# mmurooka/SMPLpp

Hardware: AMD Instinct MI355X
Metric: SMPL FK evals/s + IK iters/s, batch 1024 frames, 1/2/4/8 MI355X (higher is better)
Workload: dtype f32 (exact operands: every fp32 value as three bf16 pieces = fp32's 24 bits on the bf16 matrix pipe, fp32 accumulate; fp32 VALU skinning)

## Files before the change

smplpp_amd/csrc/skin_h.hip:

```cpp
#include "common.h"
#include "slot_pipe.h"

namespace smplpp_hip
{
typedef float f32x16 __attribute__((ext_vector_type(16)));
typedef float v3f __attribute__((ext_vector_type(3), aligned(4)));
typedef float v4f __attribute__((ext_vector_type(4)));
typedef unsigned v3u __attribute__((ext_vector_type(3)));
typedef _Float16 f16x8 __attribute__((ext_vector_type(8)));

constexpr int H_R = 7;
constexpr int H_LDS_RING = HB_G_BYTES;
constexpr int H_LDS_TR = H_LDS_RING + H_R * HB_IMG;
constexpr int H_LDS_TOTAL = H_LDS_TR + 64 * 16;

constexpr int wrap15(int u)
{
  return u < 0 ? u + HB_SLOTS : u;
}
constexpr int h_tail_slot(int k)
{
  return k <= 4 ? k : (k == 5 ? 4 : (k <= 10 ? k - 1 : (k == 11 ? 9 : k - 2)));
}
constexpr int h_tail_m(int k)
{
  return (k == 5 || k == 11) ? 8 : 5;
}
constexpr int h_tail_rows_in(int u)
{
  int c = 0;
  for(int k = 0; k < 16; k++) c += h_tail_slot(k) == u;
  return c;
}
constexpr int h_after_dma(int u, bool ht, bool rest)
{
  return u < 14 ? (ht ? h_tail_rows_in(u) : (u < 9 ? 2 : 0)) : ((u == 14 && rest) ? 16 : 0);
}
constexpr int h_slot_ops(int u, bool ht, bool rest)
{
  return 3 + h_after_dma(u, ht, rest);
}
constexpr int h_barrier_vmcnt(int s, bool ht, bool rest)
{
  if(!ht && s == 13) return 12;
  int c = s - 6 < 0 ? ((wrap15(s - 6) == 14 && rest && ht) ? 16 : 0) : h_after_dma(s - 6, ht, rest);
  for(int u = s - 5; u < s; u++) c += u < 0 ? 3 + ((wrap15(u) == 14 && rest && ht) ? 16 : 0) : h_slot_ops(u, ht, rest);
  return c < 63 ? c : 63;
}
static_assert(h_tail_rows_in(4) == 2 && h_tail_rows_in(9) == 2 && h_tail_rows_in(13) == 1 && h_tail_rows_in(14) == 0, "tail placement");
static_assert(h_barrier_vmcnt(0, false, true) == 15 && h_barrier_vmcnt(1, false, false) == 12 + 5 && h_barrier_vmcnt(0, true, true) == 31 &&
                  h_barrier_vmcnt(1, true, false) == 5 * 3 + 1 && h_barrier_vmcnt(8, true, false) == 15 + 7 && h_barrier_vmcnt(14, false, false) == 2 + 15,
              "window bookkeeping");

#ifndef SKINH_STORE_AUX
#define SKINH_STORE_AUX 0
#endif
#ifndef SKINH_DMA_IMM
#define SKINH_DMA_IMM 1
#endif
#ifndef SKINH_ABL
#define SKINH_ABL 0
#endif
#if SKINH_ABL & (256 | 512)
__device__ unsigned long long g_hslot_times[8 * 256];
__device__ unsigned long long g_hwg_times[256 * 4];
#endif

template<bool WANT_REST>
__global__ __launch_bounds__(256, 1) void skin_kernel_h(const uint8_t * __restrict__ A2h, const uint8_t * __restrict__ B2h,
                                                        const uint8_t * __restrict__ G2h, const float * __restrict__ theta,
                                                        float * __restrict__ verts, float * __restrict__ rest, int64_t n,
                                                        int64_t V, int nvg, int nft, float cAB)
{
  extern __shared__ __attribute__((aligned(16))) unsigned char lds[];
  typedef __attribute__((address_space(3))) void * lds_ptr_t;
  const int tid = threadIdx.x, lane = tid & 63, half = lane >> 5, l31 = lane & 31;
  const int wave = __builtin_amdgcn_readfirstlane(tid >> 6), wf = wave & 1, wv = wave >> 1;
  const int nbx = (int)(gridDim.x >> 3), xcd = (int)(blockIdx.x & 7), jb = (int)(blockIdx.x >> 3);
  const int vg0 = (xcd * nvg) >> 3, vg1 = ((xcd + 1) * nvg) >> 3, nvx = vg1 - vg0;
  const int cnt = nvx * nft;
  const int i0 = (int)(((unsigned)jb * (unsigned)cnt) / (unsigned)nbx), i1 = (int)(((unsigned)(jb + 1) * (unsigned)cnt) / (unsigned)nbx);
  if(i0 >= i1) return;

#if SKINH_ABL & 512
  const unsigned long long t_start = __builtin_amdgcn_s_memtime(), r_start = __builtin_amdgcn_s_memrealtime();
#endif
  const int frameB = (int)(V * 12);
  const __amdgpu_buffer_rsrc_t rsB =
      __builtin_amdgcn_make_buffer_rsrc(const_cast<uint8_t *>(B2h), 0, (int)(nvg * HB_SLOTS * HB_IMG), 0x00020000);
  const __amdgpu_buffer_rsrc_t rsG =
      __builtin_amdgcn_make_buffer_rsrc(const_cast<uint8_t *>(G2h), 0, (int)(nft * HB_G_BYTES), 0x00020000);
  const __amdgpu_buffer_rsrc_t rsV = __builtin_amdgcn_make_buffer_rsrc(verts, 0, (int)(verts ? n * V * 12 : 0), 0x00020000);
  const __amdgpu_buffer_rsrc_t rsR = __builtin_amdgcn_make_buffer_rsrc(rest, 0, (int)(rest ? n * V * 12 : 0), 0x00020000);
  const int voffDma = wave * 3072 + lane * 16;

  const unsigned char * imgV[H_R];
  int imgS[H_R];
#pragma unroll
  for(int k = 0; k < H_R; k++)
  {
    imgS[k] = H_LDS_RING + k * HB_IMG;
    imgV[k] = lds + imgS[k] + wv * 6144 + lane * 16;
  }
  const unsigned char * const gLane0 = lds + wf * (12 * 3072) + lane * 16;
  const unsigned char * const gLane1 = lds + wf * (12 * 3072) + 2048 + l31 * 16;
  const unsigned char * const trLane = lds + H_LDS_TR + (wf * 32 + 4 * half) * 16;

#if SKINH_ABL & (256 | 512)
  int dbg_item = 0;
#endif
  f32x16 acc[3], macc[3];
  float tt[3][16];
  v4f areg[HB_KS][2];
  v4f bfr[2][3][2];
  v4f gfr[2][4];
  v4f wfr[4];
  v4f trb[2];
  const f32x16 zero16 = {0.f, 0.f, 0.f, 0.f, 0.f, 0.f, 0.f, 0.f, 0.f, 0.f, 0.f, 0.f, 0.f, 0.f, 0.f, 0.f};

  struct Item
  {
    int voff;
    int sb;
    float cw;
  } cur = {0x7fffff00, 0, 0.f}, prev = {0x7fffff00, 0, 0.f};

  auto mfma = [](const v4f & a, const v4f & b, const f32x16 & c) {
    return __builtin_amdgcn_mfma_f32_32x32x16_f16(__builtin_bit_cast(f16x8, a), __builtin_bit_cast(f16x8, b), c, 0, 0, 0);
  };
  auto dma = [&](auto itag, int vgBase, int slot, int dst) {
    constexpr int I = decltype(itag)::value;
    if constexpr(SKINH_ABL & 2) return;
#if SKINH_DMA_IMM
    __builtin_amdgcn_raw_ptr_buffer_load_lds(rsB, (lds_ptr_t)(lds + dst + wave * 3072), 16, voffDma, vgBase + slot * HB_IMG, I * 1024, 0);
#else
    __builtin_amdgcn_raw_ptr_buffer_load_lds(rsB, (lds_ptr_t)(lds + dst + wave * 3072 + I * 1024), 16, voffDma,
                                             vgBase + slot * HB_IMG + I * 1024, 0, 0);
#endif
  };

  v3f ovh;
  auto tail_prep = [&](auto rtag) {
    constexpr int R = decltype(rtag)::value;
    const v4f tr = trb[R & 1];
    if constexpr(R + 1 < 16) trb[(R + 1) & 1] = *reinterpret_cast<const v4f *>(trLane + ((((R + 1) & 3) + 8 * ((R + 1) >> 2)) * 16));
    const float u = __builtin_fmaf(tt[2][R], cAB, macc[2][R]);
    ovh = v3f{__builtin_fmaf(tt[0][R], prev.cw, tr.x), __builtin_fmaf(tt[1][R], prev.cw, tr.y), __builtin_fmaf(u, prev.cw, tr.z)};
  };
  auto tail_store = [&](auto rtag) {
    constexpr int R = decltype(rtag)::value;
    constexpr int ROWC = (R & 3) + 8 * (R >> 2);
    if constexpr(SKINH_ABL & 32)
    {
      const float o0 = ovh.x, o1 = ovh.y, o2 = ovh.z;
      asm volatile("" ::"v"(o0), "v"(o1), "v"(o2));
    }
    else
      __builtin_amdgcn_raw_buffer_store_b96(__builtin_bit_cast(v3u, ovh), rsV, prev.voff, prev.sb + ROWC * frameB, SKINH_STORE_AUX);
    asm volatile("s_nop 1");
  };
  auto tail_row = [&](auto rtag) {
    tail_prep(rtag);
    tail_store(rtag);
  };
  auto standalone_tail = [&]() {
    static_for<16>([&](auto rr) {
      tail_row(rr);
      SCHED_BARRIER();
    });
  };

  auto load_frame_tile = [&](int ft, auto first_tag) {
    constexpr bool FIRST = decltype(first_tag)::value;
    full_barrier();
#if SKINH_ABL & 512
    if(FIRST && blockIdx.x == 8 && tid == 0) g_hslot_times[70] = __builtin_amdgcn_s_memtime();
#endif
    float tval = 0.0f;
    if(tid < 192)
    {
      const int64_t f = (int64_t)ft * 64 + tid / 3;
      if(f < n) tval = theta[f * ((NJ + 1) * 3) + tid % 3];
    }
    const int vgF = vg0 + i0 % nvx;
    if constexpr(FIRST)
    {
      dma(std::integral_constant<int, 0>{}, vgF * (HB_SLOTS * HB_IMG), 0, imgS[0]);
      dma(std::integral_constant<int, 1>{}, vgF * (HB_SLOTS * HB_IMG), 0, imgS[0]);
      dma(std::integral_constant<int, 2>{}, vgF * (HB_SLOTS * HB_IMG), 0, imgS[0]);
    }
    const uint8_t * ap = A2h + ((int64_t)ft * HB_KS * 2 + wf) * 2048 + lane * 16;
#pragma unroll
    for(int ks = 0; ks < HB_KS; ks++)
#pragma unroll
      for(int p = 0; p < 2; p++) areg[ks][p] = *reinterpret_cast<const v4f *>(ap + ks * HB_A_BYTES + p * 1024);
    if constexpr(FIRST)
      static_for<H_R - 1>([&](auto dd) {
        constexpr int D = decltype(dd)::value + 1;
        dma(std::integral_constant<int, 0>{}, vgF * (HB_SLOTS * HB_IMG), D, imgS[D]);
        dma(std::integral_constant<int, 1>{}, vgF * (HB_SLOTS * HB_IMG), D, imgS[D]);
        dma(std::integral_constant<int, 2>{}, vgF * (HB_SLOTS * HB_IMG), D, imgS[D]);
      });
    if constexpr(FIRST)
    {
      waitcnt_barrier<28 + 18, 0, !(SKINH_ABL & 1)>();
#pragma unroll
      for(int q = 0; q < 6; q++) bfr[0][q / 2][q % 2] = *reinterpret_cast<const v4f *>(imgV[0] + q * 1024);
    }
    if(tid < 192) *reinterpret_cast<float *>(lds + H_LDS_TR + (tid / 3) * 16 + (tid % 3) * 4) = tval;
#if SKINH_ABL & 512
    if(FIRST && blockIdx.x == 8 && tid == 0) g_hslot_times[72] = __builtin_amdgcn_s_memtime();
#endif
  };

  auto do_item = [&](int ft_in, int vg_in, int vgn_in, auto ht_tag) {
    constexpr bool HT = decltype(ht_tag)::value;
    const int ft = __builtin_amdgcn_readfirstlane(ft_in), vg = __builtin_amdgcn_readfirstlane(vg_in), vgn = __builtin_amdgcn_readfirstlane(vgn_in);
    const int Bcur = vg * (HB_SLOTS * HB_IMG), Bnext = vgn * (HB_SLOTS * HB_IMG);
    cur.sb = __builtin_amdgcn_readfirstlane((ft * 64 + wf * 32) * frameB);
    int gcls = 3;

#if SKINH_ABL & 512
    if(blockIdx.x == 8 && tid == 0 && dbg_item < 8)
    {
      g_hslot_times[dbg_item * 8 + 0] = __builtin_amdgcn_s_memtime();
      g_hslot_times[dbg_item * 8 + 1] = __builtin_amdgcn_s_memrealtime();
    }
#endif
    static_for<HB_KS>([&](auto ss) {
      constexpr int S = decltype(ss)::value;
      static_for<9>([&](auto mm) {
        constexpr int M = decltype(mm)::value, X = M / 3, Q = M % 3;
        const v4f & a = areg[S][Q == 2 ? 1 : 0];
        const v4f & b = bfr[S & 1][X][Q == 1 ? 1 : 0];
#if SKINH_ABL & 256
        if(blockIdx.x == 0 && tid == 0 && dbg_item < 8) g_hslot_times[dbg_item * 256 + S * 9 + M] = __builtin_readcyclecounter();
#endif
#if SKINH_ABL & 512
        if(M == 0 && S < 8 && blockIdx.x == 8 && tid == 0 && dbg_item == 0) g_hslot_times[80 + S] = __builtin_amdgcn_s_memtime();
#endif
        if constexpr(SKINH_ABL & 4)
        {
          if constexpr(S == 0 && Q == 0) acc[X] = zero16;
          asm volatile("" ::"v"(a), "v"(b));
        }
        else if constexpr(S == 0 && Q == 0)
          acc[X] = mfma(a, b, zero16);
        else
          acc[X] = mfma(a, b, acc[X]);
        SCHED_BARRIER();
        if constexpr(M == 1) waitcnt_barrier<h_barrier_vmcnt(S, HT, WANT_REST), 0, !(SKINH_ABL & 1)>();
        if constexpr(M >= 2 && M <= 4)
          dma(std::integral_constant<int, M - 2>{}, S + 7 < HB_SLOTS ? Bcur : Bnext, S + 7 < HB_SLOTS ? S + 7 : S + 7 - HB_SLOTS,
              imgS[S % H_R]);
        if constexpr(!HT && S < 9 && (M == 5 || M == 6))
        {
          constexpr int PC = (2 * S + (M - 5)) * 4;
          __builtin_amdgcn_raw_ptr_buffer_load_lds(rsG, (lds_ptr_t)(lds + (PC + wave) * 1024), 16, lane * 16,
                                                   ft * HB_G_BYTES + (PC + wave) * 1024, 0, 0);
        }
        if constexpr(HT && (M == 5 || M == 7))
          static_for<16>([&](auto kk) {
            constexpr int K = decltype(kk)::value;
            if constexpr(h_tail_slot(K) == S && h_tail_m(K) == (M == 5 ? 5 : 8)) tail_prep(kk);
          });
        if constexpr(HT && (M == 6 || M == 8))
          static_for<16>([&](auto kk) {
            constexpr int K = decltype(kk)::value;
            if constexpr(h_tail_slot(K) == S && h_tail_m(K) == (M == 6 ? 5 : 8)) tail_store(kk);
          });
        if constexpr(S < HB_KS - 1 && M >= 2 && M <= 4 && !(SKINH_ABL & 16))
        {
          bfr[(S + 1) & 1][M - 2][0] = *reinterpret_cast<const v4f *>(imgV[(S + 1) % H_R] + (2 * (M - 2)) * 1024);
          bfr[(S + 1) & 1][M - 2][1] = *reinterpret_cast<const v4f *>(imgV[(S + 1) % H_R] + (2 * (M - 2) + 1) * 1024);
        }
        if constexpr(S == HB_KS - 1)
        {
          const unsigned char * wimg = imgV[HB_KS % H_R] - wv * 4096;
          if constexpr(M >= 2 && M <= 5) wfr[M - 2] = *reinterpret_cast<const v4f *>(wimg + ((M - 2) / 2) * 4096 + ((M - 2) % 2) * 1024);
          if constexpr(M == 6)
          {
            cur.cw = *reinterpret_cast<const float *>(lds + imgS[HB_KS % H_R] + HB_CW_OFF + (wv * 32 + l31) * 4);
            const int pv = *reinterpret_cast<const int *>(lds + imgS[HB_KS % H_R] + HB_PERM_OFF + (wv * 32 + l31) * 4);
            cur.voff = pv >= 0 ? pv * 12 + (4 * half) * frameB : 0x7fffff00;
            gcls = __builtin_amdgcn_readfirstlane(*reinterpret_cast<const int *>(lds + imgS[HB_KS % H_R] + HB_FLAGS_OFF));
          }
          if constexpr(M == 7)
          {
            gfr[0][0] = *reinterpret_cast<const v4f *>(gLane0);
            gfr[0][1] = *reinterpret_cast<const v4f *>(gLane0 + 1024);
          }
          if constexpr(M == 8)
          {
            gfr[0][2] = *reinterpret_cast<const v4f *>(gLane1);
            gfr[0][3] = *reinterpret_cast<const v4f *>(gLane1 + 512);
          }
        }
        SCHED_BARRIER();
      });
    });

#if SKINH_ABL & 512
    if(blockIdx.x == 8 && tid == 0 && dbg_item < 8)
    {
      g_hslot_times[dbg_item * 8 + 2] = __builtin_amdgcn_s_memtime();
      g_hslot_times[dbg_item * 8 + 3] = __builtin_amdgcn_s_memrealtime();
    }
#endif
    auto skin_phase = [&](auto ctag) {
    constexpr int CLS = decltype(ctag)::value;
    constexpr bool K0 = (CLS & 1) != 0, K1 = (CLS & 2) != 0;
    static_for<12>([&](auto ee) {
      constexpr int E = decltype(ee)::value, MPE = E & 1, ME = E % 3;
      static_for<5>([&](auto bb) {
        constexpr int B = decltype(bb)::value;
        constexpr bool LIVE = (B == 0 || B == 1 || B == 3) ? K0 : K1;
        constexpr int FIRST = K0 ? 0 : 2;
        constexpr int GI = B < 2 ? 0 : (B == 2 ? 2 : (B == 3 ? 1 : 3));
        constexpr int WI = B == 0 ? 0 : (B == 1 ? 1 : (B == 2 ? 3 : (B == 3 ? 0 : 2)));
#if SKINH_ABL & 256
        if(blockIdx.x == 0 && tid == 0 && dbg_item < 8) g_hslot_times[dbg_item * 256 + 126 + E * 5 + B] = __builtin_readcyclecounter();
#endif
        if constexpr(SKINH_ABL & 8)
        {
          if constexpr(B == 0) macc[ME] = zero16;
        }
        else if constexpr(!LIVE)
          ;
        else if constexpr(B == FIRST)
          macc[ME] = mfma(gfr[MPE][GI], wfr[WI], zero16);
        else
          macc[ME] = mfma(gfr[MPE][GI], wfr[WI], macc[ME]);
        SCHED_BARRIER();
        if constexpr(E == 0 && B == 0) waitcnt_barrier<h_barrier_vmcnt(HB_KS, HT, WANT_REST), 0, !(SKINH_ABL & 1)>();
        if constexpr(E == 0 && B >= 1 && B <= 3) dma(std::integral_constant<int, B - 1>{}, Bnext, HB_KS + 7 - HB_SLOTS, imgS[HB_KS % H_R]);
        if constexpr(E == 1)
        {
          bfr[0][B / 2][B % 2] = *reinterpret_cast<const v4f *>(imgV[(HB_KS + 1) % H_R] + B * 1024);
          if constexpr(B == 4) bfr[0][2][1] = *reinterpret_cast<const v4f *>(imgV[(HB_KS + 1) % H_R] + 5 * 1024);
        }
        if constexpr(E < 11 && B <= 3 && !(SKINH_ABL & (8 | 16)))
        {
          constexpr int I = B == 0 ? 0 : (B == 1 ? 2 : (B == 2 ? 1 : 3));
          if constexpr(I < 2 ? K0 : K1)
            gfr[MPE ^ 1][I] = *reinterpret_cast<const v4f *>((I < 2 ? gLane0 + I * 1024 : gLane1 + (I - 2) * 512) + (E + 1) * 3072);
        }
        if constexpr(E == 11 && B == 4)
          trb[0] = *reinterpret_cast<const v4f *>(trLane);
        auto blend_rows = [&](auto ftag, auto r0tag, auto r1tag) {
          constexpr int F = decltype(ftag)::value, XF = F / 4, CF = F % 4, MF = F % 3, R0 = decltype(r0tag)::value, R1 = decltype(r1tag)::value;
#pragma unroll
          for(int r = R0; r < R1; r++)
          {
            if constexpr(CF == 0) tt[XF][r] = macc[MF][r] * acc[0][r];
            if constexpr(CF == 1) tt[XF][r] = __builtin_fmaf(macc[MF][r], acc[1][r], tt[XF][r]);
            if constexpr(CF == 2) tt[XF][r] = __builtin_fmaf(macc[MF][r], acc[2][r], tt[XF][r]);
            if constexpr(CF == 3) tt[XF][r] = __builtin_fmaf(tt[XF][r], cAB, macc[MF][r]);
          }
        };
        if constexpr(!(SKINH_ABL & 8))
        {
          if constexpr(E >= 1 && B >= 1)
            blend_rows(std::integral_constant<int, E - 1>{}, std::integral_constant<int, 3 * (B - 1)>{}, std::integral_constant<int, 3 * B>{});
          if constexpr(E >= 2 && B == 0)
            blend_rows(std::integral_constant<int, E - 2>{}, std::integral_constant<int, 12>{}, std::integral_constant<int, 16>{});
          if constexpr(E == 11 && B == 4)
            blend_rows(std::integral_constant<int, 10>{}, std::integral_constant<int, 12>{}, std::integral_constant<int, 16>{});
        }
        if constexpr(WANT_REST && E >= 2 && E <= 9 && B < 2)
        {
          constexpr int R = 2 * (E - 2) + B, ROWC = (R & 3) + 8 * (R >> 2);
          v3f ov = {acc[0][R] * cAB, acc[1][R] * cAB, acc[2][R] * cAB};
          __builtin_amdgcn_raw_buffer_store_b96(__builtin_bit_cast(v3u, ov), rsR, cur.voff, cur.sb + ROWC * frameB, SKINH_STORE_AUX);
          asm volatile("s_nop 1");
        }
        SCHED_BARRIER();
      });
    });
    };
    if(gcls == 1)
      skin_phase(std::integral_constant<int, 1>{});
    else if(gcls == 2)
      skin_phase(std::integral_constant<int, 2>{});
    else
      skin_phase(std::integral_constant<int, 3>{});

    prev = cur;
#if SKINH_ABL & (256 | 512)
    dbg_item++;
#endif
    {
      const unsigned char * v0 = imgV[0];
      const int s0 = imgS[0];
#pragma unroll
      for(int k = 0; k < H_R - 1; k++)
      {
        imgV[k] = imgV[k + 1];
        imgS[k] = imgS[k + 1];
      }
      imgV[H_R - 1] = v0;
      imgS[H_R - 1] = s0;
    }
  };

  for(int i = i0; i < i1;)
  {
    const int ft = i / nvx;
    const int iend = (ft + 1) * nvx < i1 ? (ft + 1) * nvx : i1;
    if(i != i0)
    {
      standalone_tail();
      load_frame_tile(ft, std::false_type{});
    }
    else
      load_frame_tile(ft, std::true_type{});
    int vgk = vg0 + (i - ft * nvx);
    auto next_vg = [&](int k, int vgc) { return k + 1 < i1 ? (vgc + 1 < vg1 ? vgc + 1 : vg0) : vgc; };
    do_item(ft, vgk, next_vg(i, vgk), std::false_type{});
    for(int k = i + 1; k < iend; k++)
    {
      vgk++;
      do_item(ft, vgk, next_vg(k, vgk), std::true_type{});
    }
    i = iend;
  }
  standalone_tail();
#if SKINH_ABL & 512
  if(blockIdx.x == 8 && tid == 0)
  {
    g_hslot_times[64] = __builtin_amdgcn_s_memtime();
    g_hslot_times[65] = __builtin_amdgcn_s_memrealtime();
    g_hslot_times[66] = t_start;
    g_hslot_times[67] = r_start;
    g_hslot_times[68] = i1 - i0;
  }
  if(tid == 0 && blockIdx.x < 256)
  {
    g_hwg_times[blockIdx.x * 4 + 0] = r_start;
    g_hwg_times[blockIdx.x * 4 + 1] = __builtin_amdgcn_s_memrealtime();
    g_hwg_times[blockIdx.x * 4 + 2] = __builtin_amdgcn_s_memtime() - t_start;
    g_hwg_times[blockIdx.x * 4 + 3] = (unsigned long long)(i1 - i0) | ((unsigned long long)__builtin_amdgcn_s_getreg((6 << 11) | 20) << 32);
  }
#endif
  asm volatile("s_waitcnt vmcnt(0)" ::: "memory");
}

static hipError_t launch_h(const smplpp_model * m, int64_t n, const float * theta, float * verts, float * rest, hipStream_t st,
                           int64_t f_off)
{
  const int nft = (int)((n + 63) / 64);
  const int nvg = (int)m->VGPn;
  const int per_xcd_items = ((nvg + 7) / 8) * nft;
  int nbx = device_cus(m->device) / 8;
  if(nbx > per_xcd_items) nbx = per_xcd_items;
  if(nbx < 1) nbx = 1;
  {
    const int rounds = (per_xcd_items + nbx - 1) / nbx;
    nbx = (per_xcd_items + rounds - 1) / rounds;
  }
  const bool wr = rest != nullptr;
  static PerDeviceOnce once[2];
  {
    hipError_t e = lds_opt_in(once[wr], m->device, wr ? reinterpret_cast<const void *>(&skin_kernel_h<true>) : reinterpret_cast<const void *>(&skin_kernel_h<false>), H_LDS_TOTAL);
    if(e != hipSuccess) return e;
  }
  const float cAB = 1.0f / (HB_SA * m->sB);
  const uint8_t * A2 = m->ws.A2h.as<uint8_t>() + (f_off / 64) * (int64_t)(HB_KS * HB_A_BYTES);
  const uint8_t * G2 = m->ws.G2h.as<uint8_t>() + (f_off / 64) * (int64_t)HB_G_BYTES;
  const float * th = theta + f_off * ((NJ + 1) * 3);
  float * vo = verts ? verts + f_off * m->V * 3 : nullptr;
  float * ro = rest ? rest + f_off * m->V * 3 : nullptr;
  if(wr)
    skin_kernel_h<true><<<dim3(nbx * 8), dim3(256), H_LDS_TOTAL, st>>>(A2, m->B2h.get(), G2, th, vo, ro, n, m->V, nvg, nft, cAB);
  else
    skin_kernel_h<false><<<dim3(nbx * 8), dim3(256), H_LDS_TOTAL, st>>>(A2, m->B2h.get(), G2, th, vo, ro, n, m->V, nvg, nft, cAB);
  return hipGetLastError();
}

#if SKINH_ABL & (256 | 512)
extern "C" int smplpp_debug_hwg_times(unsigned long long * out)
{
  return (int)hipMemcpyFromSymbol(out, HIP_SYMBOL(smplpp_hip::g_hwg_times), sizeof(unsigned long long) * 256 * 4);
}
extern "C" int smplpp_debug_hslot_times(unsigned long long * out)
{
  return (int)hipMemcpyFromSymbol(out, HIP_SYMBOL(smplpp_hip::g_hslot_times), sizeof(unsigned long long) * 8 * 256);
}
#endif
hipError_t launch_skin_f16x2(const smplpp_model * m, int64_t n, const float * theta, float * verts, float * rest, hipStream_t st)
{
  int64_t per = (0x7fffff00LL / (m->V * 12)) & ~63LL;
  const int64_t per_g = (0x7fffff00LL / HB_G_BYTES) * 64;
  if(per > per_g) per = per_g;
  if(per < 64) return hipErrorInvalidValue;
  for(int64_t off = 0; off < n; off += per)
  {
    const int64_t nn = (n - off < per) ? n - off : per;
    hipError_t e = launch_h(m, nn, theta, verts, rest, st, off);
    if(e != hipSuccess) return e;
  }
  return hipSuccess;
}
}
```

Before: 14.61 million.

## Stage A-operand loads and ring prefill progressively across first item of each run

```diff
diff --git a/smplpp_amd/csrc/skin_h.hip b/smplpp_amd/csrc/skin_h.hip
--- a/smplpp_amd/csrc/skin_h.hip
+++ b/smplpp_amd/csrc/skin_h.hip
@@ -32,25 +32,72 @@
   for(int k = 0; k < 16; k++) c += h_tail_slot(k) == u;
   return c;
 }
-constexpr int h_after_dma(int u, bool ht, bool rest)
-{
-  return u < 14 ? (ht ? h_tail_rows_in(u) : (u < 9 ? 2 : 0)) : ((u == 14 && rest) ? 16 : 0);
-}
-constexpr int h_slot_ops(int u, bool ht, bool rest)
-{
-  return 3 + h_after_dma(u, ht, rest);
-}
-constexpr int h_barrier_vmcnt(int s, bool ht, bool rest)
-{
-  if(!ht && s == 13) return 12;
-  int c = s - 6 < 0 ? ((wrap15(s - 6) == 14 && rest && ht) ? 16 : 0) : h_after_dma(s - 6, ht, rest);
-  for(int u = s - 5; u < s; u++) c += u < 0 ? 3 + ((wrap15(u) == 14 && rest && ht) ? 16 : 0) : h_slot_ops(u, ht, rest);
+#ifndef SKINH_A_PRE
+#define SKINH_A_PRE 4
+#endif
+#ifndef SKINH_RING_PRE
+#define SKINH_RING_PRE 4
+#endif
+constexpr int H_A_PRE = SKINH_A_PRE, H_RING_PRE = SKINH_RING_PRE;
+static_assert(H_A_PRE >= 1 && H_A_PRE <= HB_KS && H_RING_PRE >= 2 && H_RING_PRE <= H_R, "staging depths");
+constexpr int H_FIRST = 0, H_RUN = 1, H_TAILED = 2;
+
+constexpr bool h_moved_dma(int u, int kind)
+{
+  return kind == H_FIRST && u >= 0 && u + H_RING_PRE < H_R;
+}
+constexpr int h_a_loads(int u, int kind)
+{
+  return (kind != H_TAILED && u + H_A_PRE < HB_KS) ? 2 : 0;
+}
+constexpr int h_after_dma(int u, int kind, bool rest)
+{
+  return u < 14 ? (kind == H_TAILED ? h_tail_rows_in(u) : (u < 9 ? 2 : 0) + h_a_loads(u, kind)) : ((u == 14 && rest) ? 16 : 0);
+}
+constexpr int h_slot_ops(int u, int kind, bool rest)
+{
+  return 3 + (h_moved_dma(u, kind) ? 3 : 0) + h_after_dma(u, kind, rest);
+}
+constexpr int h_setup_after(int d)
+{
+  int c = d < H_A_PRE ? 2 : 0;
+  for(int e = d + 1; e < (H_RING_PRE > H_A_PRE ? H_RING_PRE : H_A_PRE); e++) c += (e < H_RING_PRE ? 3 : 0) + (e < H_A_PRE ? 2 : 0);
+  return c;
+}
+constexpr int h_barrier_vmcnt(int s, int kind, bool rest)
+{
+  int c = 0;
+  if(kind != H_TAILED && s + 1 < H_R)
+  {
+    if(kind == H_RUN) return 63;
+    const int u0 = s + 1 - H_RING_PRE;
+    c = u0 < 0 ? h_setup_after(s + 1) : 1 + h_after_dma(u0, kind, rest);
+    for(int u = u0 < 0 ? 0 : u0 + 1; u < s; u++) c += h_slot_ops(u, kind, rest);
+    return c < 63 ? c : 63;
+  }
+  c = s - 6 < 0 ? ((wrap15(s - 6) == 14 && rest) ? 16 : 0) : h_after_dma(s - 6, kind, rest);
+  for(int u = s - 5; u < s; u++) c += u < 0 ? 3 + ((wrap15(u) == 14 && rest) ? 16 : 0) : h_slot_ops(u, kind, rest);
+  if(kind != H_TAILED && s == 13)
+  {
+    int g = h_a_loads(8, kind);
+    for(int u = 9; u < 13; u++) g += h_slot_ops(u, kind, rest);
+    c = g < c ? g : c;
+  }
   return c < 63 ? c : 63;
 }
+constexpr int H_SETUP_VMCNT = h_setup_after(0);
 static_assert(h_tail_rows_in(4) == 2 && h_tail_rows_in(9) == 2 && h_tail_rows_in(13) == 1 && h_tail_rows_in(14) == 0, "tail placement");
-static_assert(h_barrier_vmcnt(0, false, true) == 15 && h_barrier_vmcnt(1, false, false) == 12 + 5 && h_barrier_vmcnt(0, true, true) == 31 &&
-                  h_barrier_vmcnt(1, true, false) == 5 * 3 + 1 && h_barrier_vmcnt(8, true, false) == 15 + 7 && h_barrier_vmcnt(14, false, false) == 2 + 15,
+static_assert(h_barrier_vmcnt(0, H_TAILED, true) == 31 && h_barrier_vmcnt(1, H_TAILED, false) == 5 * 3 + 1 && h_barrier_vmcnt(8, H_TAILED, false) == 15 + 7 &&
+                  h_barrier_vmcnt(14, H_TAILED, false) == 1 + 15 + 6,
               "window bookkeeping");
+static_assert(H_A_PRE != 4 || H_RING_PRE != 4 ||
+                  (H_SETUP_VMCNT == 17 && h_barrier_vmcnt(0, H_FIRST, false) == 12 && h_barrier_vmcnt(1, H_FIRST, true) == 7 + 10 &&
+                   h_barrier_vmcnt(2, H_FIRST, false) == 2 + 20 && h_barrier_vmcnt(3, H_FIRST, false) == 1 + 4 + 20 &&
+                   h_barrier_vmcnt(5, H_FIRST, false) == 1 + 4 + 14 && h_barrier_vmcnt(6, H_FIRST, false) == 4 + 41 &&
+                   h_barrier_vmcnt(7, H_FIRST, false) == 4 + 38 && h_barrier_vmcnt(7, H_RUN, false) == 4 + 35 && h_barrier_vmcnt(5, H_RUN, false) == 63 && h_barrier_vmcnt(6, H_RUN, false) == 4 + 35 &&
+                   h_barrier_vmcnt(12, H_FIRST, false) == 4 + 7 + 7 + 5 + 3 + 3 && h_barrier_vmcnt(13, H_FIRST, false) == 2 + 5 + 9 &&
+                   h_barrier_vmcnt(13, H_RUN, true) == 16 && h_barrier_vmcnt(14, H_FIRST, false) == 4 + 5 + 12 && h_barrier_vmcnt(14, H_RUN, false) == 21),
+              "window bookkeeping of a run's first item");
 
 #ifndef SKINH_STORE_AUX
 #define SKINH_STORE_AUX 0
@@ -63,7 +110,7 @@
 #endif
 #if SKINH_ABL & (256 | 512)
 __device__ unsigned long long g_hslot_times[8 * 256];
-__device__ unsigned long long g_hwg_times[256 * 4];
+__device__ unsigned long long g_hwg_times[256 * 8];
 #endif
 
 template<bool WANT_REST>
@@ -84,6 +131,7 @@
 
 #if SKINH_ABL & 512
   const unsigned long long t_start = __builtin_amdgcn_s_memtime(), r_start = __builtin_amdgcn_s_memrealtime();
+  unsigned long long t_pro = 0, t_first = 0, t_mid0 = 0, t_mid = 0, t_mid_first = 0;
 #endif
   const int frameB = (int)(V * 12);
   const __amdgpu_buffer_rsrc_t rsB =
@@ -183,27 +231,26 @@
       if(f < n) tval = theta[f * ((NJ + 1) * 3) + tid % 3];
     }
     const int vgF = vg0 + i0 % nvx;
-    if constexpr(FIRST)
-    {
-      dma(std::integral_constant<int, 0>{}, vgF * (HB_SLOTS * HB_IMG), 0, imgS[0]);
-      dma(std::integral_constant<int, 1>{}, vgF * (HB_SLOTS * HB_IMG), 0, imgS[0]);
-      dma(std::integral_constant<int, 2>{}, vgF * (HB_SLOTS * HB_IMG), 0, imgS[0]);
-    }
     const uint8_t * ap = A2h + ((int64_t)ft * HB_KS * 2 + wf) * 2048 + lane * 16;
-#pragma unroll
-    for(int ks = 0; ks < HB_KS; ks++)
-#pragma unroll
-      for(int p = 0; p < 2; p++) areg[ks][p] = *reinterpret_cast<const v4f *>(ap + ks * HB_A_BYTES + p * 1024);
-    if constexpr(FIRST)
-      static_for<H_R - 1>([&](auto dd) {
-        constexpr int D = decltype(dd)::value + 1;
+    static_for<(H_RING_PRE > H_A_PRE ? H_RING_PRE : H_A_PRE)>([&](auto dd) {
+      constexpr int D = decltype(dd)::value;
+      if constexpr(FIRST && D < H_RING_PRE)
+      {
         dma(std::integral_constant<int, 0>{}, vgF * (HB_SLOTS * HB_IMG), D, imgS[D]);
         dma(std::integral_constant<int, 1>{}, vgF * (HB_SLOTS * HB_IMG), D, imgS[D]);
         dma(std::integral_constant<int, 2>{}, vgF * (HB_SLOTS * HB_IMG), D, imgS[D]);
-      });
+      }
+      SCHED_BARRIER();
+      if constexpr(D < H_A_PRE)
+      {
+        areg[D][0] = *reinterpret_cast<const v4f *>(ap + D * HB_A_BYTES);
+        areg[D][1] = *reinterpret_cast<const v4f *>(ap + D * HB_A_BYTES + 1024);
+      }
+      SCHED_BARRIER();
+    });
     if constexpr(FIRST)
     {
-      waitcnt_barrier<28 + 18, 0, !(SKINH_ABL & 1)>();
+      waitcnt_barrier<H_SETUP_VMCNT, 0, !(SKINH_ABL & 1)>();
 #pragma unroll
       for(int q = 0; q < 6; q++) bfr[0][q / 2][q % 2] = *reinterpret_cast<const v4f *>(imgV[0] + q * 1024);
     }
@@ -213,8 +260,9 @@
 #endif
   };
 
-  auto do_item = [&](int ft_in, int vg_in, int vgn_in, auto ht_tag) {
-    constexpr bool HT = decltype(ht_tag)::value;
+  auto do_item = [&](int ft_in, int vg_in, int vgn_in, auto kind_tag) {
+    constexpr int KIND = decltype(kind_tag)::value;
+    constexpr bool HT = KIND == H_TAILED;
     const int ft = __builtin_amdgcn_readfirstlane(ft_in), vg = __builtin_amdgcn_readfirstlane(vg_in), vgn = __builtin_amdgcn_readfirstlane(vgn_in);
     const int Bcur = vg * (HB_SLOTS * HB_IMG), Bnext = vgn * (HB_SLOTS * HB_IMG);
     cur.sb = __builtin_amdgcn_readfirstlane((ft * 64 + wf * 32) * frameB);
@@ -249,10 +297,21 @@
         else
           acc[X] = mfma(a, b, acc[X]);
         SCHED_BARRIER();
-        if constexpr(M == 1) waitcnt_barrier<h_barrier_vmcnt(S, HT, WANT_REST), 0, !(SKINH_ABL & 1)>();
+        if constexpr(M == 1) waitcnt_barrier<h_barrier_vmcnt(S, KIND, WANT_REST), 0, !(SKINH_ABL & 1)>();
+        if constexpr(M >= 2 && M <= 4 && h_moved_dma(S, KIND))
+        {
+          dma(std::integral_constant<int, M - 2>{}, Bcur, S + H_RING_PRE, imgS[S + H_RING_PRE]);
+          SCHED_BARRIER();
+        }
         if constexpr(M >= 2 && M <= 4)
           dma(std::integral_constant<int, M - 2>{}, S + 7 < HB_SLOTS ? Bcur : Bnext, S + 7 < HB_SLOTS ? S + 7 : S + 7 - HB_SLOTS,
               imgS[S % H_R]);
+        if constexpr(!HT && M == 7 && S + H_A_PRE < HB_KS)
+        {
+          const uint8_t * ap = A2h + ((int64_t)ft * HB_KS * 2 + wf) * 2048 + lane * 16 + (S + H_A_PRE) * HB_A_BYTES;
+          areg[S + H_A_PRE][0] = *reinterpret_cast<const v4f *>(ap);
+          areg[S + H_A_PRE][1] = *reinterpret_cast<const v4f *>(ap + 1024);
+        }
         if constexpr(!HT && S < 9 && (M == 5 || M == 6))
         {
           constexpr int PC = (2 * S + (M - 5)) * 4;
@@ -332,7 +391,7 @@
         else
           macc[ME] = mfma(gfr[MPE][GI], wfr[WI], macc[ME]);
         SCHED_BARRIER();
-        if constexpr(E == 0 && B == 0) waitcnt_barrier<h_barrier_vmcnt(HB_KS, HT, WANT_REST), 0, !(SKINH_ABL & 1)>();
+        if constexpr(E == 0 && B == 0) waitcnt_barrier<h_barrier_vmcnt(HB_KS, KIND, WANT_REST), 0, !(SKINH_ABL & 1)>();
         if constexpr(E == 0 && B >= 1 && B <= 3) dma(std::integral_constant<int, B - 1>{}, Bnext, HB_KS + 7 - HB_SLOTS, imgS[HB_KS % H_R]);
         if constexpr(E == 1)
         {
@@ -407,20 +466,38 @@
   {
     const int ft = i / nvx;
     const int iend = (ft + 1) * nvx < i1 ? (ft + 1) * nvx : i1;
+    int vgk = vg0 + (i - ft * nvx);
+    auto next_vg = [&](int k, int vgc) { return k + 1 < i1 ? (vgc + 1 < vg1 ? vgc + 1 : vg0) : vgc; };
     if(i != i0)
     {
+#if SKINH_ABL & 512
+      t_mid0 = __builtin_amdgcn_s_memtime();
+#endif
       standalone_tail();
       load_frame_tile(ft, std::false_type{});
+#if SKINH_ABL & 512
+      t_mid = __builtin_amdgcn_s_memtime() - t_mid0;
+#endif
+      do_item(ft, vgk, next_vg(i, vgk), std::integral_constant<int, H_RUN>{});
+#if SKINH_ABL & 512
+      t_mid_first = __builtin_amdgcn_s_memtime() - t_mid0;
+#endif
     }
     else
+    {
       load_frame_tile(ft, std::true_type{});
-    int vgk = vg0 + (i - ft * nvx);
-    auto next_vg = [&](int k, int vgc) { return k + 1 < i1 ? (vgc + 1 < vg1 ? vgc + 1 : vg0) : vgc; };
-    do_item(ft, vgk, next_vg(i, vgk), std::false_type{});
+#if SKINH_ABL & 512
+      t_pro = __builtin_amdgcn_s_memtime() - t_start;
+#endif
+      do_item(ft, vgk, next_vg(i, vgk), std::integral_constant<int, H_FIRST>{});
+#if SKINH_ABL & 512
+      t_first = __builtin_amdgcn_s_memtime() - t_start;
+#endif
+    }
     for(int k = i + 1; k < iend; k++)
     {
       vgk++;
-      do_item(ft, vgk, next_vg(k, vgk), std::true_type{});
+      do_item(ft, vgk, next_vg(k, vgk), std::integral_constant<int, H_TAILED>{});
     }
     i = iend;
   }
@@ -436,10 +513,14 @@
   }
   if(tid == 0 && blockIdx.x < 256)
   {
-    g_hwg_times[blockIdx.x * 4 + 0] = r_start;
-    g_hwg_times[blockIdx.x * 4 + 1] = __builtin_amdgcn_s_memrealtime();
-    g_hwg_times[blockIdx.x * 4 + 2] = __builtin_amdgcn_s_memtime() - t_start;
-    g_hwg_times[blockIdx.x * 4 + 3] = (unsigned long long)(i1 - i0) | ((unsigned long long)__builtin_amdgcn_s_getreg((6 << 11) | 20) << 32);
+    g_hwg_times[blockIdx.x * 8 + 0] = r_start;
+    g_hwg_times[blockIdx.x * 8 + 1] = __builtin_amdgcn_s_memrealtime();
+    g_hwg_times[blockIdx.x * 8 + 2] = __builtin_amdgcn_s_memtime() - t_start;
+    g_hwg_times[blockIdx.x * 8 + 3] = (unsigned long long)(i1 - i0) | ((unsigned long long)__builtin_amdgcn_s_getreg((6 << 11) | 20) << 32);
+    g_hwg_times[blockIdx.x * 8 + 4] = t_pro;
+    g_hwg_times[blockIdx.x * 8 + 5] = t_first;
+    g_hwg_times[blockIdx.x * 8 + 6] = t_mid;
+    g_hwg_times[blockIdx.x * 8 + 7] = t_mid_first;
   }
 #endif
   asm volatile("s_waitcnt vmcnt(0)" ::: "memory");
@@ -480,7 +561,7 @@
 #if SKINH_ABL & (256 | 512)
 extern "C" int smplpp_debug_hwg_times(unsigned long long * out)
 {
-  return (int)hipMemcpyFromSymbol(out, HIP_SYMBOL(smplpp_hip::g_hwg_times), sizeof(unsigned long long) * 256 * 4);
+  return (int)hipMemcpyFromSymbol(out, HIP_SYMBOL(smplpp_hip::g_hwg_times), sizeof(unsigned long long) * 256 * 8);
 }
 extern "C" int smplpp_debug_hslot_times(unsigned long long * out)
 {
```

Result: no change. 14.78 million (median of 2 runs) (+1.2%).
